# zefanyang/pacingpseudo

Hardware: AMD Instinct MI355X
Metric: training images/sec (256x256, 5-class) (higher is better)
Workload: dtype f32 (matrix products as 3 fp16 MFMA products of split operands with fp32 accumulation, or fp32 MFMA)

## Files before the change

pacingpseudo_amd/csrc/pp_norm.hip:

```cpp
#include "pp_common.h"
#include <stdlib.h>

PP_NS_BEGIN
#define NORM_THREADS 256

struct ColPlan { int c4, rows, nblk, chunk; };

static ColPlan col_plan(int C, int Ppg, int groups) {
  ColPlan p;
  p.c4 = C / 4;
  p.rows = NORM_THREADS / p.c4;
  if (p.rows < 1) p.rows = 1;
  constexpr int blocks = 512;
  int target = blocks / groups;
  if (target < 1) target = 1;
  p.chunk = pp_cdiv(Ppg, target);
  const int min_chunk = p.rows * 8;
  if (p.chunk < min_chunk) p.chunk = min_chunk;
  p.chunk = pp_cdiv(p.chunk, p.rows) * p.rows;
  p.nblk = pp_cdiv(Ppg, p.chunk);
  return p;
}

__global__ __launch_bounds__(NORM_THREADS) void bn_stats_partial_kernel(const act_t* __restrict__ z, int ld, int C,
// ... 883 lines not shown
  if (MODE != 1) {
    __syncthreads();
    for (int c = tid; c < C; c += NORM_THREADS) {
      double a = 0.0, b = 0.0;
      const int cq2 = c >> 2, e = c & 3;
      for (int r = 0; r < rows; ++r) {
        a += (double)sh[(r * c4n + cq2) * 8 + e];
        b += (double)sh[(r * c4n + cq2) * 8 + 4 + e];
      }
      double* o = partial + ((size_t)(g * gridDim.x + blk) * 2) * C;
      o[c] = a;
      o[C + c] = b;
    }
  }
  if (MODE != 0 && amax) {
#pragma unroll
    for (int o = 32; o > 0; o >>= 1) mx = fmaxf(mx, __shfl_xor(mx, o, 64));
    if ((tid & 63) == 0 && mx > __hip_atomic_load(amax, __ATOMIC_RELAXED, __HIP_MEMORY_SCOPE_AGENT))
      atomicMax(reinterpret_cast<unsigned*>(amax), __float_as_uint(mx));
  }
}

static int bn_pool_check(const pp_act* dy, int ld_dy, const pp_act* dp, int ld_dp, const pp_act* dz, int ld_dz, int C, int B, int H,
                         int W, int groups) {
  PP_CHECK_ARG(dy && dp && dz, "bn_lrelu_bwd_pool: null pointer");
  PP_CHECK_ARG(H > 0 && W > 0 && H % 2 == 0 && W % 2 == 0 && B > 0 && groups > 0 && B % groups == 0,
               "bn_lrelu_bwd_pool: H, W must be even and groups must divide the batch (B=%d H=%d W=%d groups=%d)", B, H, W, groups);
  PP_CHECK_ARG(ld_dy % 4 == 0 && ld_dp % 4 == 0 && ld_dz % 4 == 0 && ld_dy >= C && ld_dp >= C && ld_dz >= C, "bn_lrelu_bwd_pool: bad ld");
  PP_CHECK_ARG(((((uintptr_t)dy) | ((uintptr_t)dp) | ((uintptr_t)dz)) & PP_ACT_ALIGN) == 0, "bn_lrelu_bwd_pool: tensors must be 16-byte aligned");
  return 0;
}

extern "C" int PP_FN(pp_bn_lrelu_bwd_pool)(const pp_act* dy, int ld_dy, const pp_act* dpool, int ld_dpool, const pp_act* z, int ld_z,
                                    const float* scale, const float* shift, const float* save_mean, const float* save_invstd,
                                    const float* gamma, int training, pp_act* dz, int ld_dz, float* dgamma, float* dbeta,
                                    float* dbias_conv, int accumulate_param_grads, int C, int B, int H, int W, int groups,
                                    float slope, void* workspace, size_t workspace_bytes, float* dz_amax, void* stream) {
  hipStream_t s = (hipStream_t)stream;
  const int Ppg = (B / (groups > 0 ? groups : 1)) * H * W;
  if (int rc = bn_check(z, ld_z, C, Ppg, groups)) return rc;
  if (int rc = bn_pool_check(dy, ld_dy, dpool, ld_dpool, dz, ld_dz, C, B, H, W, groups)) return rc;
  PP_CHECK_ARG(scale && shift && save_mean && save_invstd && gamma && workspace, "bn_lrelu_bwd_pool: null pointer");
  const int Wpg = Ppg / 4;
  const size_t need = pp_bn_workspace(C, Ppg, groups) + (size_t)3 * groups * C * sizeof(float);
  if (workspace_bytes < need) {
    pp_set_error("bn_lrelu_bwd_pool: workspace too small (%zu < %zu)", workspace_bytes, need);
    return PP_ERR_WORKSPACE;
  }
  ColPlan p = col_plan(C, Wpg, groups);
  double* partial = reinterpret_cast<double*>(((uintptr_t)workspace + 15) & ~(uintptr_t)15);
  float* kA = reinterpret_cast<float*>(partial + (size_t)groups * col_plan(C, Ppg, groups).nblk * 2 * C);
  float* kB = kA + (size_t)groups * C;
  float* kC = kB + (size_t)groups * C;
  pp_prof_begin(PP_K_BN, 0.0, 22.0 * (double)groups * Ppg * C, s);
  hipLaunchKernelGGL(bn_bwd_pool_kernel<0>, dim3(p.nblk, groups), dim3(NORM_THREADS), 0, s, dy, ld_dy, dpool, ld_dpool, z, ld_z,
                     scale, shift, save_mean, save_invstd, (const float*)nullptr, (const float*)nullptr, (const float*)nullptr,
                     (act_t*)nullptr, 0, C, H, W, Wpg, p.chunk, p.rows, slope, 1.0f / slope, partial, (float*)nullptr);
  hipLaunchKernelGGL(bn_bwd_finalize_kernel, dim3(pp_cdiv(C, FIN_CH)), dim3(FIN_CH * FIN_SL), 0, s, partial, p.nblk, C, Ppg,
                     groups, training, gamma, save_mean, save_invstd, kA, kB, kC, dgamma, dbeta, dbias_conv,
                     accumulate_param_grads, dz_amax);
  hipLaunchKernelGGL(bn_bwd_pool_kernel<1>, dim3(p.nblk, groups), dim3(NORM_THREADS), 0, s, dy, ld_dy, dpool, ld_dpool, z, ld_z,
                     scale, shift, (const float*)nullptr, (const float*)nullptr, kA, kB, kC, dz, ld_dz, C, H, W, Wpg, p.chunk,
                     p.rows, slope, 1.0f / slope, (double*)nullptr, dz_amax);
  pp_prof_end(s);
  return pp_launch_status("bn_lrelu_bwd_pool");
}

extern "C" int PP_FN(pp_bn_lrelu_bwd_eval_pool)(const pp_act* dy, int ld_dy, const pp_act* dpool, int ld_dpool, const pp_act* y, int ld_y,
                                         const float* scale, const float* gamma, const float* beta, pp_act* dz, int ld_dz,
                                         float* dgamma, float* dbeta, float* dbias_conv, int accumulate_param_grads, int C, int B,
                                         int H, int W, float slope, void* workspace, size_t workspace_bytes, float* dz_amax,
                                         void* stream) {
  hipStream_t s = (hipStream_t)stream;
  const int P = B * H * W;
  if (int rc = bn_check(y, ld_y, C, P, 1)) return rc;
  if (int rc = bn_pool_check(dy, ld_dy, dpool, ld_dpool, dz, ld_dz, C, B, H, W, 1)) return rc;
  PP_CHECK_ARG(scale && gamma && beta && workspace && slope > 0.f && ((uintptr_t)scale & 15) == 0, "bn_lrelu_bwd_eval_pool: bad arguments");
  if (workspace_bytes < pp_bn_workspace(C, P, 1)) {
    pp_set_error("bn_lrelu_bwd_eval_pool: workspace too small");
    return PP_ERR_WORKSPACE;
  }
  ColPlan p = col_plan(C, P / 4, 1);
  double* partial = reinterpret_cast<double*>(((uintptr_t)workspace + 15) & ~(uintptr_t)15);
  if (dz_amax && hipMemsetAsync(dz_amax, 0, sizeof(float), s) != hipSuccess) return pp_launch_status("bn_bwd_eval_pool_memset");
  pp_prof_begin(PP_K_BN, 0.0, 13.0 * (double)P * C, s);
  hipLaunchKernelGGL(bn_bwd_pool_kernel<2>, dim3(p.nblk, 1), dim3(NORM_THREADS), 0, s, dy, ld_dy, dpool, ld_dpool, y, ld_y, scale,
                     (const float*)nullptr, (const float*)nullptr, (const float*)nullptr, (const float*)nullptr,
                     (const float*)nullptr, (const float*)nullptr, dz, ld_dz, C, H, W, P / 4, p.chunk, p.rows, slope, 1.0f / slope,
                     partial, dz_amax);
  hipLaunchKernelGGL(bn_bwd_eval_finalize_kernel, dim3(pp_cdiv(C, FIN_CH)), dim3(FIN_CH * FIN_SL), 0, s, partial, p.nblk, C,
                     gamma, beta, scale, dgamma, dbeta, dbias_conv, accumulate_param_grads);
  pp_prof_end(s);
  return pp_launch_status("bn_lrelu_bwd_eval_pool");
}

__global__ __launch_bounds__(NORM_THREADS) void bn_lrelu_fwd_pool_kernel(const act_t* __restrict__ z, int ld_z, const float* __restrict__ scale,
                                                                         const float* __restrict__ shift, act_t* __restrict__ y, int ld_y,
                                                                         act_t* __restrict__ pooled, int ld_p, int C, int H, int W, int Wpg,
                                                                         int chunk, int rows, float slope) {
  const int c4n = C >> 2;
  const int tid = threadIdx.x;
  const int cq = tid % c4n, row = tid / c4n;
  if (row >= rows) return;
  const int g = blockIdx.y;
  const int w_lo = blockIdx.x * chunk;
  int w_hi = w_lo + chunk;
  if (w_hi > Wpg) w_hi = Wpg;
  const int Ho = H >> 1, Wo = W >> 1;
  const float4 sc = *reinterpret_cast<const float4*>(scale + g * C + cq * 4);
  const float4 sh = *reinterpret_cast<const float4*>(shift + g * C + cq * 4);
  const size_t img0 = (size_t)g * (Wpg / (Ho * Wo));
  for (int w = w_lo + row; w < w_hi; w += rows) {
    const int n = w / (Ho * Wo), r = w - n * (Ho * Wo), yo = r / Wo, xo = r - yo * Wo;
    const size_t p0 = ((img0 + n) * H + 2 * yo) * W + 2 * xo;
    const size_t pix[4] = {p0, p0 + 1, p0 + W, p0 + W + 1};
    float4 v[4], o[4];
#pragma unroll
    for (int i = 0; i < 4; ++i) v[i] = act_ld4f(z + pix[i] * ld_z + cq * 4);
#pragma unroll
    for (int i = 0; i < 4; ++i) {
      o[i].x = pp_lrelu(pp_bn_pre(v[i].x, sc.x, sh.x), slope);
      o[i].y = pp_lrelu(pp_bn_pre(v[i].y, sc.y, sh.y), slope);
      o[i].z = pp_lrelu(pp_bn_pre(v[i].z, sc.z, sh.z), slope);
      o[i].w = pp_lrelu(pp_bn_pre(v[i].w, sc.w, sh.w), slope);
      act_st4f(y + pix[i] * ld_y + cq * 4, o[i]);
    }
    float4 m;
    m.x = fmaxf(fmaxf(o[0].x, o[1].x), fmaxf(o[2].x, o[3].x));
    m.y = fmaxf(fmaxf(o[0].y, o[1].y), fmaxf(o[2].y, o[3].y));
    m.z = fmaxf(fmaxf(o[0].z, o[1].z), fmaxf(o[2].z, o[3].z));
    m.w = fmaxf(fmaxf(o[0].w, o[1].w), fmaxf(o[2].w, o[3].w));
    act_st4f(pooled + ((size_t)g * Wpg + w) * ld_p + cq * 4, m);
  }
}

extern "C" int PP_FN(pp_bn_lrelu_fwd_pool)(const pp_act* z, int ld_z, const float* scale, const float* shift, pp_act* y, int ld_y,
                                    pp_act* pooled, int ld_pooled, int C, int B, int H, int W, int groups, float slope, void* stream) {
  hipStream_t s = (hipStream_t)stream;
  PP_CHECK_ARG(groups > 0 && B > 0 && B % groups == 0 && H > 0 && W > 0 && H % 2 == 0 && W % 2 == 0,
               "bn_lrelu_fwd_pool: H, W must be even and groups must divide the batch");
  const int Ppg = (B / groups) * H * W;
  if (int rc = bn_check(z, ld_z, C, Ppg, groups)) return rc;
  PP_CHECK_ARG(scale && shift && y && pooled && ld_y % 4 == 0 && ld_y >= C && ld_pooled % 4 == 0 && ld_pooled >= C &&
                   ((((uintptr_t)y) | ((uintptr_t)pooled)) & PP_ACT_ALIGN) == 0, "bn_lrelu_fwd_pool: bad output");
  ColPlan p = col_plan(C, Ppg / 4, groups);
  pp_prof_begin(PP_K_BN, 0.0, 9.0 * (double)groups * Ppg * C, s);
  hipLaunchKernelGGL(bn_lrelu_fwd_pool_kernel, dim3(p.nblk, groups), dim3(NORM_THREADS), 0, s, z, ld_z, scale, shift, y, ld_y, pooled,
                     ld_pooled, C, H, W, Ppg / 4, p.chunk, p.rows, slope);
  pp_prof_end(s);
  return pp_launch_status("bn_lrelu_fwd_pool");
}
struct Wg1Args { const act_t* x; int ld_x; int H, W; float* part; };

template <bool EVAL>
__global__ __launch_bounds__(NORM_THREADS) void bn_bwd_wg1_kernel(
    const act_t* __restrict__ dy, int ld_dy, const act_t* __restrict__ zy, int ld_z, const float* __restrict__ scale,
    const float* __restrict__ shift, const float* __restrict__ kA, const float* __restrict__ kB, const float* __restrict__ kC,
    int C, int Ppg, int chunk, int rows, float slope, float inv_slope, double* __restrict__ partial, Wg1Args w) {
  __shared__ float shw[NORM_THREADS * 36];
  const int c4n = C >> 2;
  const int tid = threadIdx.x;
  const int cq = tid % c4n, row = tid / c4n;
  const bool active = row < rows;
  const int g = blockIdx.y, blk = blockIdx.x;
  const int p_lo = blk * chunk;
  int p_hi = p_lo + chunk;
  if (p_hi > Ppg) p_hi = Ppg;
  float acc[36];
#pragma unroll
  for (int k = 0; k < 36; ++k) acc[k] = 0.f;
  float s1[4] = {0, 0, 0, 0}, s2[4] = {0, 0, 0, 0};
  if (active) {
    const int co = g * C + cq * 4;
    const float4 sc = *reinterpret_cast<const float4*>(scale + co);
    float4 sf = sc, a4 = sc, b4 = sc, c4 = sc;
    if (!EVAL) {
      sf = *reinterpret_cast<const float4*>(shift + co);
      a4 = *reinterpret_cast<const float4*>(kA + co);
      b4 = *reinterpret_cast<const float4*>(kB + co);
      c4 = *reinterpret_cast<const float4*>(kC + co);
    }
    const float scv[4] = {sc.x, sc.y, sc.z, sc.w}, sfv[4] = {sf.x, sf.y, sf.z, sf.w};
    const float av[4] = {a4.x, a4.y, a4.z, a4.w}, bv[4] = {b4.x, b4.y, b4.z, b4.w}, cv[4] = {c4.x, c4.y, c4.z, c4.w};
    const size_t gb = (size_t)g * Ppg;
    const act_t* dyb = dy + gb * ld_dy + cq * 4;
    const act_t* zb = zy + gb * ld_z + cq * 4;
    const act_t* xb = w.x + gb * w.ld_x;
    int p = p_lo + row;
    int xx = p % w.W, yy = (p / w.W) % w.H;
    const int dxx = rows % w.W, dyy = rows / w.W;
    auto step = [&]() __attribute__((always_inline)) {
      p += rows; xx += dxx; yy += dyy;
      if (xx >= w.W) { xx -= w.W; ++yy; }
      if (yy >= w.H) yy -= w.H;
      if (yy >= w.H) yy %= w.H;
    };
    auto load = [&](float4& d4, float4& z4, float (&xs)[9]) __attribute__((always_inline)) {
      d4 = act_ld4f(dyb + (size_t)p * ld_dy);
      z4 = act_ld4f(zb + (size_t)p * ld_z);
#pragma unroll
      for (int t = 0; t < 9; ++t) {
        const int oy = t / 3 - 1, ox = t % 3 - 1;
        const bool ok = (unsigned)(yy + oy) < (unsigned)w.H && (unsigned)(xx + ox) < (unsigned)w.W;
        const float v = act_ld1(xb + (size_t)(ok ? p + oy * w.W + ox : p) * w.ld_x);
        xs[t] = ok ? v : 0.f;
      }
    };
    auto consume = [&](const float4& d4, const float4& z4, const float (&xs)[9]) __attribute__((always_inline)) {
      const float dv[4] = {d4.x, d4.y, d4.z, d4.w}, zv[4] = {z4.x, z4.y, z4.z, z4.w};
#pragma unroll
      for (int e = 0; e < 4; ++e) {
        float o;
        if (EVAL) {
          const bool pos = zv[e] > 0.f;
          const float gg = pos ? dv[e] : dv[e] * slope;
          const float pre = pos ? zv[e] : zv[e] * inv_slope;
          s1[e] += gg;
          s2[e] += gg * pre;
          o = scv[e] * gg;
        } else {
          o = av[e] * (pp_bn_pre(zv[e], scv[e], sfv[e]) > 0.f ? dv[e] : dv[e] * slope) + bv[e] * zv[e] + cv[e];
        }
#pragma unroll
        for (int t = 0; t < 9; ++t) acc[e * 9 + t] = __builtin_fmaf(o, xs[t], acc[e * 9 + t]);
      }
    };
    float4 d0, z0, d1, z1;
    float x0[9], x1[9];
    while (p + rows < p_hi) {
      load(d0, z0, x0); step();
      load(d1, z1, x1); step();
      consume(d0, z0, x0);
      consume(d1, z1, x1);
    }
    if (p < p_hi) {
      load(d0, z0, x0);
      consume(d0, z0, x0);
    }
#pragma unroll
    for (int k = 0; k < 36; ++k) shw[(row * c4n + cq) * 36 + k] = acc[k];
  }
  __syncthreads();
  const int n_out = C * 9;
  for (int idx = tid; idx < n_out; idx += NORM_THREADS) {
    const int o = idx / 9, t = idx - o * 9, cq2 = o >> 2, e = o & 3;
    double a = 0.0;
    for (int r = 0; r < rows; ++r) a += (double)shw[(r * c4n + cq2) * 36 + e * 9 + t];
    w.part[(size_t)(g * gridDim.x + blk) * n_out + idx] = (float)a;
  }
  if (EVAL) {
    __syncthreads();
    if (active) {
      float* d = shw + (row * c4n + cq) * 8;
#pragma unroll
      for (int e = 0; e < 4; ++e) { d[e] = s1[e]; d[4 + e] = s2[e]; }
    }
    __syncthreads();
    for (int c = tid; c < C; c += NORM_THREADS) {
      double a = 0.0, b = 0.0;
      const int cq2 = c >> 2, e = c & 3;
      for (int r = 0; r < rows; ++r) {
        a += (double)shw[(r * c4n + cq2) * 8 + e];
        b += (double)shw[(r * c4n + cq2) * 8 + 4 + e];
      }
      double* o = partial + ((size_t)blk * 2) * C;
      o[c] = a;
      o[C + c] = b;
    }
  }
}

__global__ __launch_bounds__(FIN_CH * FIN_SL) void wg1_finalize_kernel(const float* __restrict__ part, int nslab, int n_out,
                                                                      float* __restrict__ dw, int accumulate) {
  __shared__ double red[FIN_SL][FIN_CH];
  const int cl = threadIdx.x & (FIN_CH - 1), slice = threadIdx.x / FIN_CH;
  const int idx = blockIdx.x * FIN_CH + cl;
  double a = 0.0;
  if (idx < n_out)
    for (int sl = slice; sl < nslab; sl += FIN_SL) a += (double)part[(size_t)sl * n_out + idx];
  red[slice][cl] = a;
  __syncthreads();
  if (slice == 0 && idx < n_out) {
    double t = 0.0;
#pragma unroll
    for (int i = 0; i < FIN_SL; ++i) t += red[i][cl];
    dw[idx] = (accumulate ? dw[idx] : 0.f) + (float)t;
  }
}

static ColPlan wg1_plan(int C, int Ppg, int groups) {
  ColPlan p = col_plan(C, Ppg, groups);
  constexpr int blocks = 1024;
  int target = blocks / groups;
  if (target < 1) target = 1;
  p.chunk = pp_cdiv(Ppg, target);
  if (p.chunk < p.rows * 8) p.chunk = p.rows * 8;
  p.chunk = pp_cdiv(p.chunk, p.rows) * p.rows;
  p.nblk = pp_cdiv(Ppg, p.chunk);
  return p;
}

extern "C" size_t PP_FN(pp_bn_lrelu_bwd_wgrad_c1_workspace)(int C, int P_per_group, int groups) {
  ColPlan p = col_plan(C, P_per_group, groups), q = wg1_plan(C, P_per_group, groups);
  const int nb = p.nblk > q.nblk ? p.nblk : q.nblk;
  return (size_t)groups * nb * 2 * C * sizeof(double) + 256 + (size_t)3 * groups * C * sizeof(float) +
         (size_t)groups * q.nblk * C * 9 * sizeof(float) + 64;
}

static int wg1_check(const void* x, int ld_x, int H, int W, int P_per_group, const float* dw, int C, const void* workspace,
                     size_t workspace_bytes, size_t need) {
  PP_CHECK_ARG(x && dw && workspace && ld_x >= 1 && H > 0 && W > 0 && P_per_group % (H * W) == 0,
               "bn_lrelu_bwd_wgrad_c1: x / dw / workspace null, or a group is not a whole number of H x W images");
  PP_CHECK_ARG(C % 4 == 0 && C <= 4 * NORM_THREADS, "bn_lrelu_bwd_wgrad_c1: C=%d", C);
  if (workspace_bytes < need) {
    pp_set_error("bn_lrelu_bwd_wgrad_c1: workspace too small (%zu < %zu)", workspace_bytes, need);
    return PP_ERR_WORKSPACE;
  }
  return 0;
}

extern "C" int PP_FN(pp_bn_lrelu_bwd_wgrad_c1)(const pp_act* dy, int ld_dy, const pp_act* z, int ld_z, const float* scale,
                                        const float* shift, const float* save_mean, const float* save_invstd,
                                        const float* gamma, int training, const pp_act* x, int ld_x, int H, int W,
                                        float* dw_o1hw, int accumulate_dw, float* dgamma, float* dbeta, float* dbias_conv,
                                        int accumulate_param_grads, int C, int P_per_group, int groups, float slope,
                                        void* workspace, size_t workspace_bytes, void* stream) {
  hipStream_t s = (hipStream_t)stream;
  if (int rc = bn_check(z, ld_z, C, P_per_group, groups)) return rc;
  PP_CHECK_ARG(dy && scale && shift && save_mean && save_invstd && gamma, "bn_lrelu_bwd_wgrad_c1: null pointer");
  PP_CHECK_ARG(ld_dy % 4 == 0 && ld_dy >= C && ((uintptr_t)dy & PP_ACT_ALIGN) == 0, "bn_lrelu_bwd_wgrad_c1: bad dy");
  if (int rc = wg1_check(x, ld_x, H, W, P_per_group, dw_o1hw, C, workspace, workspace_bytes,
                         PP_FN(pp_bn_lrelu_bwd_wgrad_c1_workspace)(C, P_per_group, groups))) return rc;
  ColPlan p = col_plan(C, P_per_group, groups), q = wg1_plan(C, P_per_group, groups);
  double* partial = reinterpret_cast<double*>(((uintptr_t)workspace + 15) & ~(uintptr_t)15);
  float* kA = reinterpret_cast<float*>(partial + (size_t)groups * (p.nblk > q.nblk ? p.nblk : q.nblk) * 2 * C);
  float* kB = kA + (size_t)groups * C;
  float* kC = kB + (size_t)groups * C;
  float* part = kC + (size_t)groups * C;
  pp_prof_begin(PP_K_BN, 0.0, 16.0 * (double)groups * P_per_group * C, s);
  hipLaunchKernelGGL(bn_bwd_partial_kernel, dim3(p.nblk, groups), dim3(NORM_THREADS), 0, s, dy, ld_dy, z, ld_z, scale,
                     shift, save_mean, save_invstd, C, P_per_group, p.chunk, p.rows, slope, partial);
  hipLaunchKernelGGL(bn_bwd_finalize_kernel, dim3(pp_cdiv(C, FIN_CH)), dim3(FIN_CH * FIN_SL), 0, s, partial, p.nblk, C, P_per_group,
                     groups, training, gamma, save_mean, save_invstd, kA, kB, kC, dgamma, dbeta, dbias_conv,
                     accumulate_param_grads, (float*)nullptr);
  hipLaunchKernelGGL(bn_bwd_wg1_kernel<false>, dim3(q.nblk, groups), dim3(NORM_THREADS), 0, s, dy, ld_dy, z, ld_z, scale, shift,
                     kA, kB, kC, C, P_per_group, q.chunk, q.rows, slope, 1.0f / slope, (double*)nullptr, Wg1Args{x, ld_x, H, W, part});
  hipLaunchKernelGGL(wg1_finalize_kernel, dim3(pp_cdiv(C * 9, FIN_CH)), dim3(FIN_CH * FIN_SL), 0, s, part, groups * q.nblk, C * 9,
                     dw_o1hw, accumulate_dw);
  pp_prof_end(s);
  return pp_launch_status("bn_lrelu_bwd_wgrad_c1");
}

extern "C" int PP_FN(pp_bn_lrelu_bwd_eval_wgrad_c1)(const pp_act* dy, int ld_dy, const pp_act* y, int ld_y, const float* scale,
                                             const float* gamma, const float* beta, const pp_act* x, int ld_x, int H, int W,
                                             float* dw_o1hw, int accumulate_dw, float* dgamma, float* dbeta,
                                             float* dbias_conv, int accumulate_param_grads, int C, int P_total, float slope,
                                             void* workspace, size_t workspace_bytes, void* stream) {
  hipStream_t s = (hipStream_t)stream;
  if (int rc = bn_check(y, ld_y, C, P_total, 1)) return rc;
  PP_CHECK_ARG(dy && scale && gamma && beta && slope > 0.f, "bn_lrelu_bwd_eval_wgrad_c1: null pointer / slope");
  PP_CHECK_ARG(ld_dy % 4 == 0 && ld_dy >= C && ((uintptr_t)dy & PP_ACT_ALIGN) == 0 && ((uintptr_t)scale & 15) == 0,
               "bn_lrelu_bwd_eval_wgrad_c1: bad dy / scale");
  if (int rc = wg1_check(x, ld_x, H, W, P_total, dw_o1hw, C, workspace, workspace_bytes,
                         PP_FN(pp_bn_lrelu_bwd_wgrad_c1_workspace)(C, P_total, 1))) return rc;
  ColPlan p0 = col_plan(C, P_total, 1), p = wg1_plan(C, P_total, 1);
  double* partial = reinterpret_cast<double*>(((uintptr_t)workspace + 15) & ~(uintptr_t)15);
  float* part = reinterpret_cast<float*>(partial + (size_t)(p.nblk > p0.nblk ? p.nblk : p0.nblk) * 2 * C) + (size_t)3 * C;
  pp_prof_begin(PP_K_BN, 0.0, 8.0 * (double)P_total * C, s);
  hipLaunchKernelGGL(bn_bwd_wg1_kernel<true>, dim3(p.nblk, 1), dim3(NORM_THREADS), 0, s, dy, ld_dy, y, ld_y, scale, scale, scale,
                     scale, scale, C, P_total, p.chunk, p.rows, slope, 1.0f / slope, partial, Wg1Args{x, ld_x, H, W, part});
  hipLaunchKernelGGL(bn_bwd_eval_finalize_kernel, dim3(pp_cdiv(C, FIN_CH)), dim3(FIN_CH * FIN_SL), 0, s, partial, p.nblk, C,
                     gamma, beta, scale, dgamma, dbeta, dbias_conv, accumulate_param_grads);
  hipLaunchKernelGGL(wg1_finalize_kernel, dim3(pp_cdiv(C * 9, FIN_CH)), dim3(FIN_CH * FIN_SL), 0, s, part, p.nblk, C * 9, dw_o1hw,
                     accumulate_dw);
  pp_prof_end(s);
  return pp_launch_status("bn_lrelu_bwd_eval_wgrad_c1");
}
#ifndef PP_ACT_16
#define GN_THREADS 256

__device__ __forceinline__ void gn_block_sum2(double (*red)[GN_THREADS], double& a, double& b) {
  const int tid = threadIdx.x;
  red[0][tid] = a;
  red[1][tid] = b;
  __syncthreads();
#pragma unroll
  for (int o = GN_THREADS / 2; o > 0; o >>= 1) {
    if (tid < o) { red[0][tid] += red[0][tid + o]; red[1][tid] += red[1][tid + o]; }
    __syncthreads();
  }
  a = red[0][0];
  b = red[1][0];
}

__global__ __launch_bounds__(GN_THREADS) void gn_stats_finalize_kernel(const double* __restrict__ partial, int nblk, int C, int G,
                                                                     int HW, float eps, const float* __restrict__ gamma,
                                                                     const float* __restrict__ beta, float* __restrict__ save_mean,
                                                                     float* __restrict__ save_invstd, float* __restrict__ save_xbar,
                                                                     float* __restrict__ scale, float* __restrict__ shift) {
  __shared__ double red[2][GN_THREADS];
  const int g = blockIdx.x, n = blockIdx.y, tid = threadIdx.x;
  const int cpg = C / G, c0 = g * cpg;
  const double* pn = partial + (size_t)n * nblk * 2 * C;
  double s = 0.0, q = 0.0;
  for (int i = tid; i < nblk * cpg; i += GN_THREADS) {
    const int blk = i / cpg, c = c0 + (i - blk * cpg);
    s += pn[(size_t)blk * 2 * C + c];
    q += pn[(size_t)blk * 2 * C + C + c];
  }
  gn_block_sum2(red, s, q);
  const double m = (double)cpg * HW;
  const double mean = s / m;
  double var = q / m - mean * mean;
  if (var < 0.0) var = 0.0;
  const float meanf = (float)mean;
  const float invstd = 1.0f / sqrtf((float)var + eps);
  for (int cc = tid; cc < cpg; cc += GN_THREADS) {
    const int c = c0 + cc;
    double cs = 0.0;
    for (int blk = 0; blk < nblk; ++blk) cs += pn[(size_t)blk * 2 * C + c];
    const float sc = invstd * gamma[c];
    const size_t o = (size_t)n * C + c;
    save_mean[o] = meanf;
    save_invstd[o] = invstd;
    save_xbar[o] = (float)((cs / (double)HW - mean) * (double)invstd);
    scale[o] = sc;
    shift[o] = beta[c] - meanf * sc;
  }
}

__global__ __launch_bounds__(GN_THREADS) void gn_bwd_finalize_kernel(const double* __restrict__ partial, int nblk, int C, int G, int HW,
                                                                   const float* __restrict__ gamma, const float* __restrict__ mean,
                                                                   const float* __restrict__ invstd, const float* __restrict__ xbar,
                                                                   float* __restrict__ kA, float* __restrict__ kB,
                                                                   float* __restrict__ kC, double* __restrict__ rows,
                                                                   float* __restrict__ amax) {
  __shared__ double red[2][GN_THREADS];
  const int g = blockIdx.x, n = blockIdx.y, tid = threadIdx.x;
  if (amax && g == 0 && n == 0 && tid == 0) *amax = 0.f;
  const int cpg = C / G, c0 = g * cpg;
  const double* pn = partial + (size_t)n * nblk * 2 * C;
  double* rn = rows + (size_t)n * 3 * C;
  double a1 = 0.0, a2 = 0.0;
  for (int cc = tid; cc < cpg; cc += GN_THREADS) {
    const int c = c0 + cc;
    double s1 = 0.0, s2 = 0.0;
    for (int blk = 0; blk < nblk; ++blk) {
      s1 += pn[(size_t)blk * 2 * C + c];
      s2 += pn[(size_t)blk * 2 * C + C + c];
    }
    rn[c] = s1;
    rn[C + c] = s2;
    a1 += (double)gamma[c] * s1;
    a2 += (double)gamma[c] * s2;
  }
  gn_block_sum2(red, a1, a2);
  const double m = (double)cpg * HW;
  for (int cc = tid; cc < cpg; cc += GN_THREADS) {
    const int c = c0 + cc;
    const size_t o = (size_t)n * C + c;
    const double r = (double)invstd[o];
    const double A = (double)gamma[c] * r;
    const double B = -r * r * a2 / m;
    kA[o] = (float)A;
    kB[o] = (float)B;
    kC[o] = (float)(-r * a1 / m - B * (double)mean[o]);
    rn[2 * C + c] = r * ((double)gamma[c] * rn[c] - (double)HW * a1 / m - (double)HW * (double)xbar[o] * a2 / m);
  }
}

__global__ void gn_param_grads_kernel(const double* __restrict__ rows, int C, int N, float* dgamma, float* dbeta, float* dbias,
                                      int accumulate) {
  const int c = blockIdx.x * blockDim.x + threadIdx.x;
  if (c >= C) return;
  double db = 0.0, dg = 0.0, dbc = 0.0;
  for (int n = 0; n < N; ++n) {
    const double* rn = rows + (size_t)n * 3 * C;
    db += rn[c];
    dg += rn[C + c];
    dbc += rn[2 * C + c];
  }
  if (dgamma) dgamma[c] = (accumulate ? dgamma[c] : 0.f) + (float)dg;
  if (dbeta) dbeta[c] = (accumulate ? dbeta[c] : 0.f) + (float)db;
  if (dbias) dbias[c] = (accumulate ? dbias[c] : 0.f) + (float)dbc;
}

extern "C" size_t pp_gn_workspace(int C, int HW, int N) {
  return pp_bn_workspace(C, HW, N) + (size_t)N * 3 * C * sizeof(double) + (size_t)3 * N * C * sizeof(float) + 64;
}

static int gn_check(const float* z, int ld, int C, int HW, int N, int G, const void* workspace, size_t workspace_bytes,
                    const char* who) {
  if (int rc = bn_check(z, ld, C, HW, N)) return rc;
  PP_CHECK_ARG(G > 0 && C % G == 0, "%s: G=%d must divide C=%d", who, G, C);
  PP_CHECK_ARG(workspace != nullptr, "%s: null workspace", who);
  if (workspace_bytes < pp_gn_workspace(C, HW, N)) {
    pp_set_error("%s: workspace too small (%zu < %zu)", who, workspace_bytes, pp_gn_workspace(C, HW, N));
    return PP_ERR_WORKSPACE;
  }
  return 0;
}

struct GnWs { double* partial; double* rows; float *kA, *kB, *kC; };

static GnWs gn_ws(void* workspace, int C, int HW, int N) {
  GnWs w;
  w.partial = reinterpret_cast<double*>(((uintptr_t)workspace + 15) & ~(uintptr_t)15);
  w.rows = w.partial + (size_t)N * col_plan(C, HW, N).nblk * 2 * C;
  w.kA = reinterpret_cast<float*>(w.rows + (size_t)N * 3 * C);
  w.kB = w.kA + (size_t)N * C;
  w.kC = w.kB + (size_t)N * C;
  return w;
}

extern "C" int pp_gn_stats(const float* z, int ld, int C, int HW, int N, int G, float eps, const float* gamma, const float* beta,
                           float* save_mean, float* save_invstd, float* save_xbar, float* scale, float* shift, void* workspace,
                           size_t workspace_bytes, void* stream) {
  hipStream_t s = (hipStream_t)stream;
  if (int rc = gn_check(z, ld, C, HW, N, G, workspace, workspace_bytes, "gn_stats")) return rc;
  PP_CHECK_ARG(gamma && beta && save_mean && save_invstd && save_xbar && scale && shift, "gn_stats: null pointer");
  ColPlan p = col_plan(C, HW, N);
  GnWs w = gn_ws(workspace, C, HW, N);
  pp_prof_begin(PP_K_BN, 0.0, 4.0 * (double)N * HW * C, s);
// ... 61 lines not shown
```

Before: 1043.

## Fuse BN backward statistics and first-layer wgrad into a single sums pass

```diff
diff --git a/pacingpseudo_amd/csrc/pp_norm.hip b/pacingpseudo_amd/csrc/pp_norm.hip
--- a/pacingpseudo_amd/csrc/pp_norm.hip
+++ b/pacingpseudo_amd/csrc/pp_norm.hip
@@ -1059,11 +1059,35 @@
 }
 struct Wg1Args { const act_t* x; int ld_x; int H, W; float* part; };
 
-template <bool EVAL>
-__global__ __launch_bounds__(NORM_THREADS) void bn_bwd_wg1_kernel(
-    const act_t* __restrict__ dy, int ld_dy, const act_t* __restrict__ zy, int ld_z, const float* __restrict__ scale,
-    const float* __restrict__ shift, const float* __restrict__ kA, const float* __restrict__ kB, const float* __restrict__ kC,
-    int C, int Ppg, int chunk, int rows, float slope, float inv_slope, double* __restrict__ partial, Wg1Args w) {
+struct Wg1Walk {
+  const act_t *dyb, *zb, *xb;
+  int ld_dy, ld_z, ld_x, H, W, rows, dxx, dyy, p, xx, yy;
+  __device__ __forceinline__ Wg1Walk(const act_t* dy, int ld_dy_, const act_t* z, int ld_z_, const Wg1Args& w, size_t gb, int cq, int p0,
+                                     int rows_)
+      : dyb(dy + gb * ld_dy_ + cq * 4), zb(z + gb * ld_z_ + cq * 4), xb(w.x + gb * w.ld_x), ld_dy(ld_dy_), ld_z(ld_z_), ld_x(w.ld_x),
+        H(w.H), W(w.W), rows(rows_), dxx(rows_ % w.W), dyy(rows_ / w.W), p(p0), xx(p0 % w.W), yy((p0 / w.W) % w.H) {}
+  __device__ __forceinline__ void step() {
+    p += rows; xx += dxx; yy += dyy;
+    if (xx >= W) { xx -= W; ++yy; }
+    if (yy >= H) yy -= H;
+    if (yy >= H) yy %= H;
+  }
+  __device__ __forceinline__ void load(float4& d4, float4& z4, float (&xs)[9]) const {
+    d4 = act_ld4f(dyb + (size_t)p * ld_dy);
+    z4 = act_ld4f(zb + (size_t)p * ld_z);
+#pragma unroll
+    for (int t = 0; t < 9; ++t) {
+      const int oy = t / 3 - 1, ox = t % 3 - 1;
+      const bool ok = (unsigned)(yy + oy) < (unsigned)H && (unsigned)(xx + ox) < (unsigned)W;
+      const float v = act_ld1(xb + (size_t)(ok ? p + oy * W + ox : p) * ld_x);
+      xs[t] = ok ? v : 0.f;
+    }
+  }
+};
+
+__global__ __launch_bounds__(NORM_THREADS) void bn_bwd_eval_wg1_kernel(
+    const act_t* __restrict__ dy, int ld_dy, const act_t* __restrict__ y, int ld_y, const float* __restrict__ scale, int C, int Ppg,
+    int chunk, int rows, float slope, float inv_slope, double* __restrict__ partial, Wg1Args w) {
   __shared__ float shw[NORM_THREADS * 36];
   const int c4n = C >> 2;
   const int tid = threadIdx.x;
@@ -1078,70 +1102,33 @@
   for (int k = 0; k < 36; ++k) acc[k] = 0.f;
   float s1[4] = {0, 0, 0, 0}, s2[4] = {0, 0, 0, 0};
   if (active) {
-    const int co = g * C + cq * 4;
-    const float4 sc = *reinterpret_cast<const float4*>(scale + co);
-    float4 sf = sc, a4 = sc, b4 = sc, c4 = sc;
-    if (!EVAL) {
-      sf = *reinterpret_cast<const float4*>(shift + co);
-      a4 = *reinterpret_cast<const float4*>(kA + co);
-      b4 = *reinterpret_cast<const float4*>(kB + co);
-      c4 = *reinterpret_cast<const float4*>(kC + co);
-    }
-    const float scv[4] = {sc.x, sc.y, sc.z, sc.w}, sfv[4] = {sf.x, sf.y, sf.z, sf.w};
-    const float av[4] = {a4.x, a4.y, a4.z, a4.w}, bv[4] = {b4.x, b4.y, b4.z, b4.w}, cv[4] = {c4.x, c4.y, c4.z, c4.w};
-    const size_t gb = (size_t)g * Ppg;
-    const act_t* dyb = dy + gb * ld_dy + cq * 4;
-    const act_t* zb = zy + gb * ld_z + cq * 4;
-    const act_t* xb = w.x + gb * w.ld_x;
-    int p = p_lo + row;
-    int xx = p % w.W, yy = (p / w.W) % w.H;
-    const int dxx = rows % w.W, dyy = rows / w.W;
-    auto step = [&]() __attribute__((always_inline)) {
-      p += rows; xx += dxx; yy += dyy;
-      if (xx >= w.W) { xx -= w.W; ++yy; }
-      if (yy >= w.H) yy -= w.H;
-      if (yy >= w.H) yy %= w.H;
-    };
-    auto load = [&](float4& d4, float4& z4, float (&xs)[9]) __attribute__((always_inline)) {
-      d4 = act_ld4f(dyb + (size_t)p * ld_dy);
-      z4 = act_ld4f(zb + (size_t)p * ld_z);
-#pragma unroll
-      for (int t = 0; t < 9; ++t) {
-        const int oy = t / 3 - 1, ox = t % 3 - 1;
-        const bool ok = (unsigned)(yy + oy) < (unsigned)w.H && (unsigned)(xx + ox) < (unsigned)w.W;
-        const float v = act_ld1(xb + (size_t)(ok ? p + oy * w.W + ox : p) * w.ld_x);
-        xs[t] = ok ? v : 0.f;
-      }
-    };
+    const float4 sc = *reinterpret_cast<const float4*>(scale + g * C + cq * 4);
+    const float scv[4] = {sc.x, sc.y, sc.z, sc.w};
+    Wg1Walk wk(dy, ld_dy, y, ld_y, w, (size_t)g * Ppg, cq, p_lo + row, rows);
     auto consume = [&](const float4& d4, const float4& z4, const float (&xs)[9]) __attribute__((always_inline)) {
       const float dv[4] = {d4.x, d4.y, d4.z, d4.w}, zv[4] = {z4.x, z4.y, z4.z, z4.w};
 #pragma unroll
       for (int e = 0; e < 4; ++e) {
-        float o;
-        if (EVAL) {
-          const bool pos = zv[e] > 0.f;
-          const float gg = pos ? dv[e] : dv[e] * slope;
-          const float pre = pos ? zv[e] : zv[e] * inv_slope;
-          s1[e] += gg;
-          s2[e] += gg * pre;
-          o = scv[e] * gg;
-        } else {
-          o = av[e] * (pp_bn_pre(zv[e], scv[e], sfv[e]) > 0.f ? dv[e] : dv[e] * slope) + bv[e] * zv[e] + cv[e];
-        }
+        const bool pos = zv[e] > 0.f;
+        const float gg = pos ? dv[e] : dv[e] * slope;
+        const float pre = pos ? zv[e] : zv[e] * inv_slope;
+        s1[e] += gg;
+        s2[e] += gg * pre;
+        const float o = scv[e] * gg;
 #pragma unroll
         for (int t = 0; t < 9; ++t) acc[e * 9 + t] = __builtin_fmaf(o, xs[t], acc[e * 9 + t]);
       }
     };
     float4 d0, z0, d1, z1;
     float x0[9], x1[9];
-    while (p + rows < p_hi) {
-      load(d0, z0, x0); step();
-      load(d1, z1, x1); step();
+    while (wk.p + rows < p_hi) {
+      wk.load(d0, z0, x0); wk.step();
+      wk.load(d1, z1, x1); wk.step();
       consume(d0, z0, x0);
       consume(d1, z1, x1);
     }
-    if (p < p_hi) {
-      load(d0, z0, x0);
+    if (wk.p < p_hi) {
+      wk.load(d0, z0, x0);
       consume(d0, z0, x0);
     }
 #pragma unroll
@@ -1155,24 +1142,184 @@
     for (int r = 0; r < rows; ++r) a += (double)shw[(r * c4n + cq2) * 36 + e * 9 + t];
     w.part[(size_t)(g * gridDim.x + blk) * n_out + idx] = (float)a;
   }
-  if (EVAL) {
+  __syncthreads();
+  if (active) {
+    float* d = shw + (row * c4n + cq) * 8;
+#pragma unroll
+    for (int e = 0; e < 4; ++e) { d[e] = s1[e]; d[4 + e] = s2[e]; }
+  }
+  __syncthreads();
+  for (int c = tid; c < C; c += NORM_THREADS) {
+    double a = 0.0, b = 0.0;
+    const int cq2 = c >> 2, e = c & 3;
+    for (int r = 0; r < rows; ++r) {
+      a += (double)shw[(r * c4n + cq2) * 8 + e];
+      b += (double)shw[(r * c4n + cq2) * 8 + 4 + e];
+    }
+    double* o = partial + ((size_t)blk * 2) * C;
+    o[c] = a;
+    o[C + c] = b;
+  }
+}
+
+__host__ __device__ static inline size_t wg1_sums_row(int C) { return (size_t)20 * C + 16; }
+
+template <bool TRAIN>
+__global__ __launch_bounds__(NORM_THREADS) void bn_bwd_wg1_sums_kernel(
+    const act_t* __restrict__ dy, int ld_dy, const act_t* __restrict__ z, int ld_z, const float* __restrict__ scale,
+    const float* __restrict__ shift, const float* __restrict__ mean, const float* __restrict__ invstd, int C, int Ppg, int chunk,
+    int rows, float slope, double* __restrict__ partial, Wg1Args w) {
+  __shared__ float shw[NORM_THREADS * 36];
+  const int c4n = C >> 2;
+  const int tid = threadIdx.x;
+  const int cq = tid % c4n, row = tid / c4n;
+  const bool active = row < rows;
+  const int g = blockIdx.y, blk = blockIdx.x;
+  const int p_lo = blk * chunk;
+  int p_hi = p_lo + chunk;
+  if (p_hi > Ppg) p_hi = Ppg;
+  float agx[36], axx[36], sx[9];
+#pragma unroll
+  for (int k = 0; k < 36; ++k) agx[k] = axx[k] = 0.f;
+#pragma unroll
+  for (int t = 0; t < 9; ++t) sx[t] = 0.f;
+  float s1[4] = {0, 0, 0, 0}, s2[4] = {0, 0, 0, 0};
+  if (active) {
+    const int co = g * C + cq * 4;
+    const float4 sc = *reinterpret_cast<const float4*>(scale + co);
+    const float4 sf = *reinterpret_cast<const float4*>(shift + co);
+    const float4 mu = *reinterpret_cast<const float4*>(mean + co);
+    const float4 is = *reinterpret_cast<const float4*>(invstd + co);
+    const float scv[4] = {sc.x, sc.y, sc.z, sc.w}, sfv[4] = {sf.x, sf.y, sf.z, sf.w};
+    const float muv[4] = {mu.x, mu.y, mu.z, mu.w}, isv[4] = {is.x, is.y, is.z, is.w};
+    Wg1Walk wk(dy, ld_dy, z, ld_z, w, (size_t)g * Ppg, cq, p_lo + row, rows);
+    auto consume = [&](const float4& d4, const float4& z4, const float (&xs)[9]) __attribute__((always_inline)) {
+      const float dv[4] = {d4.x, d4.y, d4.z, d4.w}, zv[4] = {z4.x, z4.y, z4.z, z4.w};
+#pragma unroll
+      for (int e = 0; e < 4; ++e) {
+        const float gg = pp_bn_pre(zv[e], scv[e], sfv[e]) > 0.f ? dv[e] : dv[e] * slope;
+        const float xh = (zv[e] - muv[e]) * isv[e];
+        s1[e] += gg;
+        s2[e] += gg * xh;
+#pragma unroll
+        for (int t = 0; t < 9; ++t) {
+          agx[e * 9 + t] = __builtin_fmaf(gg, xs[t], agx[e * 9 + t]);
+          if (TRAIN) axx[e * 9 + t] = __builtin_fmaf(xh, xs[t], axx[e * 9 + t]);
+        }
+      }
+      if (TRAIN)
+#pragma unroll
+        for (int t = 0; t < 9; ++t) sx[t] += xs[t];
+    };
+    float4 d0, z0, d1, z1;
+    float x0[9], x1[9];
+    while (wk.p + rows < p_hi) {
+      wk.load(d0, z0, x0); wk.step();
+      wk.load(d1, z1, x1); wk.step();
+      consume(d0, z0, x0);
+      consume(d1, z1, x1);
+    }
+    if (wk.p < p_hi) {
+      wk.load(d0, z0, x0);
+      consume(d0, z0, x0);
+    }
+  }
+  double* prow = partial + (size_t)(g * gridDim.x + blk) * wg1_sums_row(C);
+  const int n_out = C * 9;
+  auto reduce36 = [&](const float (&a)[36], double* out) __attribute__((always_inline)) {
+    if (active)
+#pragma unroll
+      for (int k = 0; k < 36; ++k) shw[(row * c4n + cq) * 36 + k] = a[k];
     __syncthreads();
-    if (active) {
-      float* d = shw + (row * c4n + cq) * 8;
-#pragma unroll
-      for (int e = 0; e < 4; ++e) { d[e] = s1[e]; d[4 + e] = s2[e]; }
+    for (int idx = tid; idx < n_out; idx += NORM_THREADS) {
+      const int o = idx / 9, t = idx - o * 9, cq2 = o >> 2, e = o & 3;
+      double v = 0.0;
+      for (int r = 0; r < rows; ++r) v += (double)shw[(r * c4n + cq2) * 36 + e * 9 + t];
+      out[idx] = v;
     }
     __syncthreads();
-    for (int c = tid; c < C; c += NORM_THREADS) {
-      double a = 0.0, b = 0.0;
-      const int cq2 = c >> 2, e = c & 3;
-      for (int r = 0; r < rows; ++r) {
-        a += (double)shw[(r * c4n + cq2) * 8 + e];
-        b += (double)shw[(r * c4n + cq2) * 8 + 4 + e];
+  };
+  reduce36(agx, prow);
+  if (TRAIN) reduce36(axx, prow + n_out);
+  if (active) {
+    float* d = shw + (row * c4n + cq) * 17;
+#pragma unroll
+    for (int e = 0; e < 4; ++e) { d[e] = s1[e]; d[4 + e] = s2[e]; }
+#pragma unroll
+    for (int t = 0; t < 9; ++t) d[8 + t] = sx[t];
+  }
+  __syncthreads();
+  for (int c = tid; c < C; c += NORM_THREADS) {
+    double a = 0.0, b = 0.0;
+    const int cq2 = c >> 2, e = c & 3;
+    for (int r = 0; r < rows; ++r) {
+      a += (double)shw[(r * c4n + cq2) * 17 + e];
+      b += (double)shw[(r * c4n + cq2) * 17 + 4 + e];
+    }
+    prow[2 * n_out + c] = a;
+    prow[2 * n_out + C + c] = b;
+  }
+  if (TRAIN && tid < 9) {
+    double a = 0.0;
+    for (int r = 0; r < rows; ++r) a += (double)shw[(r * c4n) * 17 + 8 + tid];
+    prow[2 * n_out + 2 * C + tid] = a;
+  }
+}
+
+__global__ __launch_bounds__(FIN_CH * FIN_SL) void wg1_sums_finalize_kernel(const double* __restrict__ partial, int nblk, int C, int Ppg,
+                                                                           int groups, int training, const float* gamma,
+                                                                           const float* invstd, float* __restrict__ dw,
+                                                                           int accumulate_dw, float* dgamma, float* dbeta, float* dbias,
+                                                                           int accumulate) {
+  __shared__ double red[FIN_SL][FIN_CH][5];
+  const int cl = threadIdx.x & (FIN_CH - 1), slice = threadIdx.x / FIN_CH;
+  const int n_out = C * 9;
+  const int idx = blockIdx.x * FIN_CH + cl;
+  const bool valid = idx < n_out;
+  const int o = valid ? idx / 9 : 0, t = valid ? idx - o * 9 : 0;
+  const size_t row = wg1_sums_row(C);
+  const double n = (double)Ppg;
+  double dwv = 0.0, dg = 0.0, db = 0.0, dbc = 0.0;
+  for (int g = 0; g < groups; ++g) {
+    double v[5] = {0.0, 0.0, 0.0, 0.0, 0.0};
+    if (valid)
+      for (int blk = slice; blk < nblk; blk += FIN_SL) {
+        const double* r = partial + (size_t)(g * nblk + blk) * row;
+        v[0] += r[idx];
+        v[2] += r[2 * n_out + o];
+        v[3] += r[2 * n_out + C + o];
+        if (training) {
+          v[1] += r[n_out + idx];
+          v[4] += r[2 * n_out + 2 * C + t];
+        }
       }
-      double* o = partial + ((size_t)blk * 2) * C;
-      o[c] = a;
-      o[C + c] = b;
+    __syncthreads();
+#pragma unroll
+    for (int k = 0; k < 5; ++k) red[slice][cl][k] = v[k];
+    __syncthreads();
+    if (slice != 0 || !valid) continue;
+#pragma unroll
+    for (int k = 0; k < 5; ++k) v[k] = 0.0;
+#pragma unroll 4
+    for (int i = 0; i < FIN_SL; ++i)
+#pragma unroll
+      for (int k = 0; k < 5; ++k) v[k] += red[i][cl][k];
+    const double A = (double)gamma[o] * (double)invstd[g * C + o];
+    dg += v[3];
+    db += v[2];
+    if (training) {
+      dwv += A * (v[0] - (v[3] / n) * v[1] - (v[2] / n) * v[4]);
+    } else {
+      dwv += A * v[0];
+      dbc += A * v[2];
+    }
+  }
+  if (slice == 0 && valid) {
+    dw[idx] = (accumulate_dw ? dw[idx] : 0.f) + (float)dwv;
+    if (t == 0) {
+      if (dgamma) dgamma[o] = (accumulate ? dgamma[o] : 0.f) + (float)dg;
+      if (dbeta) dbeta[o] = (accumulate ? dbeta[o] : 0.f) + (float)db;
+      if (dbias) dbias[o] = (accumulate ? dbias[o] : 0.f) + (float)dbc;
     }
   }
 }
@@ -1195,9 +1342,8 @@
   }
 }
 
-static ColPlan wg1_plan(int C, int Ppg, int groups) {
+static ColPlan wg1_plan(int C, int Ppg, int groups, int blocks = 1024 ) {
   ColPlan p = col_plan(C, Ppg, groups);
-  constexpr int blocks = 1024;
   int target = blocks / groups;
   if (target < 1) target = 1;
   p.chunk = pp_cdiv(Ppg, target);
@@ -1207,11 +1353,15 @@
   return p;
 }
 
+constexpr int WG1_SUMS_BLOCKS = 1024;
+
 extern "C" size_t PP_FN(pp_bn_lrelu_bwd_wgrad_c1_workspace)(int C, int P_per_group, int groups) {
   ColPlan p = col_plan(C, P_per_group, groups), q = wg1_plan(C, P_per_group, groups);
   const int nb = p.nblk > q.nblk ? p.nblk : q.nblk;
-  return (size_t)groups * nb * 2 * C * sizeof(double) + 256 + (size_t)3 * groups * C * sizeof(float) +
-         (size_t)groups * q.nblk * C * 9 * sizeof(float) + 64;
+  const size_t eval_form = (size_t)groups * nb * 2 * C * sizeof(double) + 256 + (size_t)3 * groups * C * sizeof(float) +
+                           (size_t)groups * q.nblk * C * 9 * sizeof(float) + 64;
+  const size_t train_form = (size_t)groups * wg1_plan(C, P_per_group, groups, WG1_SUMS_BLOCKS).nblk * wg1_sums_row(C) * sizeof(double) + 256;
+  return eval_form > train_form ? eval_form : train_form;
 }
 
 static int wg1_check(const void* x, int ld_x, int H, int W, int P_per_group, const float* dw, int C, const void* workspace,
@@ -1238,22 +1388,18 @@
   PP_CHECK_ARG(ld_dy % 4 == 0 && ld_dy >= C && ((uintptr_t)dy & PP_ACT_ALIGN) == 0, "bn_lrelu_bwd_wgrad_c1: bad dy");
   if (int rc = wg1_check(x, ld_x, H, W, P_per_group, dw_o1hw, C, workspace, workspace_bytes,
                          PP_FN(pp_bn_lrelu_bwd_wgrad_c1_workspace)(C, P_per_group, groups))) return rc;
-  ColPlan p = col_plan(C, P_per_group, groups), q = wg1_plan(C, P_per_group, groups);
+  ColPlan q = wg1_plan(C, P_per_group, groups, WG1_SUMS_BLOCKS);
   double* partial = reinterpret_cast<double*>(((uintptr_t)workspace + 15) & ~(uintptr_t)15);
-  float* kA = reinterpret_cast<float*>(partial + (size_t)groups * (p.nblk > q.nblk ? p.nblk : q.nblk) * 2 * C);
-  float* kB = kA + (size_t)groups * C;
-  float* kC = kB + (size_t)groups * C;
-  float* part = kC + (size_t)groups * C;
-  pp_prof_begin(PP_K_BN, 0.0, 16.0 * (double)groups * P_per_group * C, s);
-  hipLaunchKernelGGL(bn_bwd_partial_kernel, dim3(p.nblk, groups), dim3(NORM_THREADS), 0, s, dy, ld_dy, z, ld_z, scale,
-                     shift, save_mean, save_invstd, C, P_per_group, p.chunk, p.rows, slope, partial);
-  hipLaunchKernelGGL(bn_bwd_finalize_kernel, dim3(pp_cdiv(C, FIN_CH)), dim3(FIN_CH * FIN_SL), 0, s, partial, p.nblk, C, P_per_group,
-                     groups, training, gamma, save_mean, save_invstd, kA, kB, kC, dgamma, dbeta, dbias_conv,
-                     accumulate_param_grads, (float*)nullptr);
-  hipLaunchKernelGGL(bn_bwd_wg1_kernel<false>, dim3(q.nblk, groups), dim3(NORM_THREADS), 0, s, dy, ld_dy, z, ld_z, scale, shift,
-                     kA, kB, kC, C, P_per_group, q.chunk, q.rows, slope, 1.0f / slope, (double*)nullptr, Wg1Args{x, ld_x, H, W, part});
-  hipLaunchKernelGGL(wg1_finalize_kernel, dim3(pp_cdiv(C * 9, FIN_CH)), dim3(FIN_CH * FIN_SL), 0, s, part, groups * q.nblk, C * 9,
-                     dw_o1hw, accumulate_dw);
+  const Wg1Args w{x, ld_x, H, W, nullptr};
+  pp_prof_begin(PP_K_BN, 0.0, (double)groups * P_per_group * (8.0 * C + 4.0), s);
+  if (training)
+    hipLaunchKernelGGL(bn_bwd_wg1_sums_kernel<true>, dim3(q.nblk, groups), dim3(NORM_THREADS), 0, s, dy, ld_dy, z, ld_z, scale, shift,
+                       save_mean, save_invstd, C, P_per_group, q.chunk, q.rows, slope, partial, w);
+  else
+    hipLaunchKernelGGL(bn_bwd_wg1_sums_kernel<false>, dim3(q.nblk, groups), dim3(NORM_THREADS), 0, s, dy, ld_dy, z, ld_z, scale, shift,
+                       save_mean, save_invstd, C, P_per_group, q.chunk, q.rows, slope, partial, w);
+  hipLaunchKernelGGL(wg1_sums_finalize_kernel, dim3(pp_cdiv(C * 9, FIN_CH)), dim3(FIN_CH * FIN_SL), 0, s, partial, q.nblk, C, P_per_group,
+                     groups, training, gamma, save_invstd, dw_o1hw, accumulate_dw, dgamma, dbeta, dbias_conv, accumulate_param_grads);
   pp_prof_end(s);
   return pp_launch_status("bn_lrelu_bwd_wgrad_c1");
 }
@@ -1274,8 +1420,8 @@
   double* partial = reinterpret_cast<double*>(((uintptr_t)workspace + 15) & ~(uintptr_t)15);
   float* part = reinterpret_cast<float*>(partial + (size_t)(p.nblk > p0.nblk ? p.nblk : p0.nblk) * 2 * C) + (size_t)3 * C;
   pp_prof_begin(PP_K_BN, 0.0, 8.0 * (double)P_total * C, s);
-  hipLaunchKernelGGL(bn_bwd_wg1_kernel<true>, dim3(p.nblk, 1), dim3(NORM_THREADS), 0, s, dy, ld_dy, y, ld_y, scale, scale, scale,
-                     scale, scale, C, P_total, p.chunk, p.rows, slope, 1.0f / slope, partial, Wg1Args{x, ld_x, H, W, part});
+  hipLaunchKernelGGL(bn_bwd_eval_wg1_kernel, dim3(p.nblk, 1), dim3(NORM_THREADS), 0, s, dy, ld_dy, y, ld_y, scale, C, P_total,
+                     p.chunk, p.rows, slope, 1.0f / slope, partial, Wg1Args{x, ld_x, H, W, part});
   hipLaunchKernelGGL(bn_bwd_eval_finalize_kernel, dim3(pp_cdiv(C, FIN_CH)), dim3(FIN_CH * FIN_SL), 0, s, partial, p.nblk, C,
                      gamma, beta, scale, dgamma, dbeta, dbias_conv, accumulate_param_grads);
   hipLaunchKernelGGL(wg1_finalize_kernel, dim3(pp_cdiv(C * 9, FIN_CH)), dim3(FIN_CH * FIN_SL), 0, s, part, p.nblk, C * 9, dw_o1hw,
```

Result: no change. 1046 (median of 6 runs) (+0.3%).
